# IDEA-Research/MP-Former

Measured on AMD Instinct MI355X. Metric: training images/sec COCO-instance R50 1024x1024, higher is better.
Workload: dtype bf16 (backbone, decoder) + f32 (pixel decoder, losses), as the reference's AMP; 1 GPU; COCO-instance R50, 100 queries, 80 classes, 1024x1024: full train step = R50 backbone + MSDeformAttn pixel decoder (6 layers) + MP masked decoder (9 layers, NUM_DN 1) + Hungarian matching + 60 losses + backward + grad all-reduce + clip + AdamW; head_only_workload=False, global_batch=2, per_gpu_batch=2, parallelism=dp1, msda_offsets=init, full=False, autograd_threads=backward on the launch thread, miopen_find_db=shipped

## Files before the change

### include/mpformer_hip.h

```cpp
#ifndef MPFORMER_HIP_H
#define MPFORMER_HIP_H

#include <stddef.h>
#include <stdint.h>

#ifdef __cplusplus
extern "C" {
#endif

enum { MPF_F32 = 0, MPF_F64 = 1, MPF_BF16 = 2, MPF_U8 = 3, MPF_BITS = 4  };

enum {
    MPF_OK = 0,
    MPF_E_DTYPE = -1,
    MPF_E_SHAPE = -2,
    MPF_E_NULL = -3,
    MPF_E_TOO_LARGE = -4
};

int mpf_abi_version(void);
const char* mpf_last_error(void);

int mpf_msda_forward(const void* value, const int64_t* spatial_shapes,
                     const int64_t* level_start_index, const void* sampling_loc,
// ... 244 lines not shown
    int N, Q, HW, pad;
    float eps;
} MpfNextMask;
size_t mpf_next_attn_mask_scratch_bytes(int N, int Q);
int mpf_next_attn_mask(const MpfNextMask* m, void* stream);
int mpf_decoder_layer_backward(const MpfDecoderLayer* layer, const MpfDecoderLayerGrad* grad, void* stream);

typedef struct MpfScaleCastItem {
    const void* src;
    void* dst;
    const float* scale;
    int64_t numel, inner, first_block;
} MpfScaleCastItem;

int mpf_grouped_scale_cast(const MpfScaleCastItem* items_device, int n_items, int64_t total_blocks, int src_dtype, int dst_dtype,
                           void* stream);

#define MPF_AMAX_SLOT_FLOATS 512
int mpf_res_ln256_forward_b(const float* x, const void* t, int t_dtype, const float* gamma, const float* beta, float* s_out, float* y32,
                            void* y16, float* mean, float* rstd, int rows, float eps, const float* padd, int padd_rows, float* y_plus,
                            float* y_bound, const float* padd_amax, float* yplus_bound, void* stream);
int mpf_res_ln256_backward_ws_amax(const float* s, const float* mean, const float* rstd, const float* gamma, const float* gy32,
                                   const void* gy16, const float* gy_plus, float* ds32, void* ds16, float* dgamma, float* dbeta, int rows,
                                   void* workspace, size_t workspace_bytes, float* ds_amax, void* stream);
typedef struct MpfAmaxItem {
    const float* src;
    float* out;
    int64_t numel, first_block;
} MpfAmaxItem;
typedef struct MpfSplitItemH2 {
    const float* src;
    void* dst;
    const float* amax;
    int64_t rows, cols, transpose, dst_ld, plane_stride, first_block;
} MpfSplitItemH2;
int mpf_amax_f32(const float* x, int64_t n, float* amax, void* stream);
int mpf_amax_f32_grouped(const MpfAmaxItem* items_device, int n_items, int64_t total_blocks, void* stream);
int mpf_h2_range_stats(const float* a, int rows, int cols, int64_t lda, const float* amax_slot, int log2_below,
                       unsigned long long* counters_device, void* stream);
int mpf_gemm3_split_grouped_h2(const MpfSplitItemH2* items_device, int n_items, int64_t total_blocks, void* stream);
typedef struct MpfNtItemH2 {
    const float* a;
    int64_t lda;
    const float* a_amax;
    const float* b;
    int64_t ldb;
    const float* b_amax;
    float* c_part;
    float* csum_a;
    int64_t Mdim, Ndim;
} MpfNtItemH2;
int mpf_gemm3_nt_h2(const float* a, int64_t lda, const float* a_amax, const float* b, int64_t ldb, const float* b_amax,
                    float* c_part, float* csum_a, float* csum_b, int R, int Mdim, int Ndim, int rows_per_split,
                    int transpose_out, void* stream);
int mpf_gemm3_nt_grouped_h2(const MpfNtItemH2* items, int n_items, int R, int rows_per_split, int64_t split_stride, void* stream);
int mpf_gemm3_conv3x3_h2(const float* x, const float* x_amax, const void* w_planes_h2, const float* w_amax, const float* bias,
                         float* y, float* out_amax, int n_img, int H, int W, int Cin, int Cout, int transposed, void* stream);
int mpf_gemm3_conv3x3_wgrad_h2(const float* dy, const float* dy_amax, const float* x, const float* x_amax, float* c_part,
                               float* csum_dy, int n_img, int H, int W, int Cin, int Cout, int rows_per_split, void* stream);
int mpf_gemm3_tn_h2(const float* a, int64_t lda, const float* a_amax, const void* b_planes_h2, const float* b_amax,
                    const float* bias, const float* c_in, int64_t ldcin, const float* c_in2, int64_t ldcin2,
                    const float* gate, int64_t ldgate, float* c, int64_t ldc, float* out_amax, int M, int N, int K,
                    int relu, void* stream);
int mpf_gemm3_tn_h2_bits(const float* a, int64_t lda, const float* a_amax, const void* b_planes_h2, const float* b_amax,
                         const float* bias, const float* c_in, int64_t ldcin, const float* c_in2, int64_t ldcin2,
                         const unsigned char* gate_bits, int64_t ldgbits, float* c, int64_t ldc, float* out_amax,
                         unsigned char* gate_bits_out, int64_t ldgbits_out, int M, int N, int K, int relu, void* stream);

typedef struct MpfNtItem {
    const float* a;
    int64_t lda;
    const float* b;
    int64_t ldb;
    float* c_part;
    float* csum_a;
    int64_t Mdim, Ndim;
} MpfNtItem;
int mpf_gemm3_nt_grouped(const MpfNtItem* items, int n_items, int R, int rows_per_split, int64_t split_stride, void* stream);

int mpf_gemm3_conv3x3(const float* x, const void* w_planes, const float* bias, float* y, int n_img, int H, int W, int Cin,
                      int Cout, int transposed, void* stream);
int mpf_gemm3_conv3x3_wgrad(const float* dy, const float* x, float* c_part, float* csum_dy, int n_img, int H, int W, int Cin, int Cout,
                            int rows_per_split, void* stream);

int mpf_gemm3_tn_ex(const void* a, int a_dtype, int64_t lda, const void* b_planes, const float* bias, const float* c_in, int64_t ldcin,
                    void* c, int c_dtype, int64_t ldc, int M, int N, int K, int relu, void* stream);
int mpf_gemm3_nt_ex(const void* a, int a_dtype, int64_t lda, const void* b, int b_dtype, int64_t ldb, float* c_part, float* csum_a,
                    int R, int Mdim, int Ndim, int rows_per_split, void* stream);

typedef struct MpfSplitItem {
    const float* src;
    void* dst;
    int64_t rows, cols, transpose, dst_ld, plane_stride, first_block;
} MpfSplitItem;

int mpf_gemm3_split_grouped(const MpfSplitItem* items_device, int n_items, int64_t total_blocks, void* stream);

typedef struct MpfOptItem {
    float* param;
    const float* grad;
    float* exp_avg;
    float* exp_avg_sq;
    int64_t numel, first_block;
    float lr, weight_decay, bc1, bc2_sqrt;
} MpfOptItem;

int mpf_clip_adamw_step(const MpfOptItem* items_device, int n_items, int64_t total_blocks, float max_norm, double beta1,
                        double beta2, double eps, float* partial, float* norm_clip, void* stream);

int mpf_transpose_f32(const float* in, int64_t in_batch_stride, float* out, int64_t out_batch_stride, int B, int R, int C,
                      void* stream);

int mpf_gemm3_nt_reduce(const float* c_part, int64_t c_numel, const float* s_part, int64_t s_numel, int nsplit,
                        float* c_out, float* s_out, void* stream);
int mpf_gemm3_nt_reduce_levels(const float* c_part, int64_t c_numel, const float* s_part, int64_t s_numel, int nsplit,
                               const int64_t* level_of_split, int n_levels, float* c_out, float* lvl_out, float* s_out, void* stream);

int mpf_tall_gemm_bf16(const void* a, int64_t lda, const void* b, int64_t ldb, const void* bias, void* c, int64_t ldc, int M, int N,
                       int K, void* stream);
size_t mpf_gemm_nt_bf16_workspace_bytes(int R, int Mdim, int Ndim, int rows_per_split);
int mpf_gemm_nt_bf16(const void* a, int64_t lda, const void* b, int64_t ldb, void* c_out, void* csum_out, int R, int Mdim,
                     int Ndim, int rows_per_split, void* workspace, size_t workspace_bytes, void* stream);

int mpf_small_gemm_bf16_blocked(const void* a, int64_t a_rs, int64_t a_ks, int a_blk, int64_t a_bs, const void* gate, const void* b,
                                int64_t b_rs, int64_t b_ks, const void* bias, const void* c_in, int64_t ldcin, void* c, int64_t ldc,
                                int c_blk, int64_t c_bs, void* rowsum_a, int I, int J, int Kc, int relu, void* stream);

int mpf_class_loss_forward(const void* logits, int dtype, int64_t sl, int64_t sn, int64_t sq, const int64_t* target,
                           int target_per_output, const float* weight, int L, int N, int Q, int C, float* lse, float* ce,
                           float* wsum, void* stream);
int mpf_class_loss_backward(const void* logits, int dtype, int64_t sl, int64_t sn, int64_t sq, const int64_t* target,
                            int target_per_output, const float* weight, int L, int N, int Q, int C, const float* lse,
                            const float* wsum, const float* grad_ce, void* dlogits, void* stream);
int mpf_mask_loss_finalize(const float* sums, const int64_t* runs, const float* norm, int n, int G, int points, float* out,
                           void* stream);
int mpf_mask_loss_finalize_backward(const float* sums, const int64_t* runs, const float* norm, int n, int G, int points,
                                    const float* grad_out, float* dsums, void* stream);

typedef struct {
    const void* a;
    const void* gate;
    const void* b;
    void* c;
    void* rowsum_a;
    int64_t a_rs, a_ks, a_bs, b_rs, b_ks, ldc;
    int a_blk, I, J, Kc;
} MpfSmallGemmItem;
int mpf_small_gemm_bf16_group(const MpfSmallGemmItem* items, int n_items, void* stream);
typedef struct MpfTransposeItem {
    const void* src;
    const void* gate;
    void* dst;
    int64_t ld;
    int R, C;
} MpfTransposeItem;
int mpf_transpose_group_bf16(const MpfTransposeItem* items, int n_items, int Rp, void* stream);

int mpf_bias_act(const void* x, const float* bias, const void* res, void* y, int64_t numel, int C, int dtype,
                 int relu, void* stream);
int mpf_relu_bwd_add(const void* ga, const void* gb, const void* y, void* out, int64_t numel, int dtype, void* stream);
int mpf_maxpool3x3s2_forward(const void* x, void* y, void* code, int N, int H, int W, int C, void* stream);
int mpf_maxpool3x3s2_backward(const void* gy, const void* code, void* gx, int N, int H, int W, int C, void* stream);

int mpf_upload_small(const void* host_src, void* device_dst, int64_t nbytes, void* stream);

int mpf_res_ln256_forward(const float* x, const void* t, int t_dtype, const float* gamma, const float* beta,
// ... 144 lines not shown
```

### mp_former_amd/_lib.py

```python
import ctypes

import torch
import os

_HERE = os.path.dirname(os.path.abspath(__file__))
LIB_PATH = os.path.join(_HERE, "libmpformer_hip.so")
LIB_PATH = os.environ.get("MPF_LIB_PATH", LIB_PATH)
ABI_VERSION = 1

MPF_F32, MPF_F64, MPF_BF16, MPF_U8, MPF_BITS = 0, 1, 2, 3, 4
DTYPE = {torch.float32: MPF_F32, torch.float64: MPF_F64, torch.bfloat16: MPF_BF16, torch.uint8: MPF_U8, torch.bool: MPF_U8}

_lib = None
_status_fns = {}

_c_int = ctypes.c_int
_c_vp = ctypes.c_void_p

SIGNATURES = {
    "mpf_abi_version": (_c_int, []),
    "mpf_last_error": (ctypes.c_char_p, []),
    "mpf_last_kernel": (ctypes.c_char_p, []),
    "mpf_set_option": (_c_int, [ctypes.c_char_p, _c_int]),
    "mpf_match_cost_fused_workspace_bytes": (ctypes.c_size_t, [_c_int] * 5),
# ... 49 lines not shown
    "mpf_amax_f32": (_c_int, [_c_vp, ctypes.c_int64, _c_vp, _c_vp]),
    "mpf_amax_f32_grouped": (_c_int, [_c_vp, _c_int, ctypes.c_int64, _c_vp]),
    "mpf_h2_range_stats": (_c_int, [_c_vp, _c_int, _c_int, ctypes.c_int64, _c_vp, _c_int, _c_vp, _c_vp]),
    "mpf_gemm3_split_grouped_h2": (_c_int, [_c_vp, _c_int, ctypes.c_int64, _c_vp]),
    "mpf_gemm3_tn_h2": (_c_int, [_c_vp, ctypes.c_int64, _c_vp, _c_vp, _c_vp, _c_vp, _c_vp, ctypes.c_int64, _c_vp, ctypes.c_int64,
                              _c_vp, ctypes.c_int64, _c_vp, ctypes.c_int64, _c_vp, _c_int, _c_int, _c_int, _c_int, _c_vp]),
    "mpf_gemm3_tn_h2_bits": (_c_int, [_c_vp, ctypes.c_int64, _c_vp, _c_vp, _c_vp, _c_vp, _c_vp, ctypes.c_int64, _c_vp, ctypes.c_int64,
                                   _c_vp, ctypes.c_int64, _c_vp, ctypes.c_int64, _c_vp, _c_vp, ctypes.c_int64,
                                   _c_int, _c_int, _c_int, _c_int, _c_vp]),
    "mpf_gemm3_nt_h2": (_c_int, [_c_vp, ctypes.c_int64, _c_vp, _c_vp, ctypes.c_int64, _c_vp, _c_vp, _c_vp, _c_vp,
                              _c_int, _c_int, _c_int, _c_int, _c_int, _c_vp]),
    "mpf_gemm3_nt_grouped_h2": (_c_int, [_c_vp, _c_int, _c_int, _c_int, ctypes.c_int64, _c_vp]),
    "mpf_gemm3_conv3x3_h2": (_c_int, [_c_vp] * 7 + [_c_int] * 6 + [_c_vp]),
    "mpf_gemm3_conv3x3_wgrad_h2": (_c_int, [_c_vp, _c_vp, _c_vp, _c_vp, _c_vp, _c_vp, _c_int, _c_int, _c_int, _c_int, _c_int, _c_int, _c_vp]),
    "mpf_gemm3_nt_grouped": (_c_int, [_c_vp, _c_int, _c_int, _c_int, ctypes.c_int64, _c_vp]),
    "mpf_small_gemm_bf16": (_c_int, [_c_vp, ctypes.c_int64, ctypes.c_int64, _c_vp, _c_vp, ctypes.c_int64, ctypes.c_int64, _c_vp, _c_vp,
                                     ctypes.c_int64, _c_vp, ctypes.c_int64, _c_vp, _c_int, _c_int, _c_int, _c_int, _c_vp]),
    "mpf_encoder_fields": (_c_int, []),
    "mpf_encoder_forward": (_c_int, [_c_vp, _c_vp]),
    "mpf_encoder_bwd_fields": (_c_int, []),
    "mpf_encoder_backward": (_c_int, [_c_vp, _c_vp]),
    "mpf_decoder_layer_struct_bytes": (ctypes.c_uint64, [_c_int]),
    "mpf_decoder_layer_scratch_bytes": (ctypes.c_uint64, [_c_int] * 6),
    "mpf_decoder_layer_forward": (_c_int, [_c_vp, _c_vp]),
    "mpf_next_attn_mask_scratch_bytes": (ctypes.c_size_t, [_c_int, _c_int]),
    "mpf_next_attn_mask": (_c_int, [_c_vp, _c_vp]),
    "mpf_lin256_res_ln_forward": (_c_int, [_c_vp] * 11 + [_c_int, ctypes.c_float, _c_vp]),
    "mpf_ln256_mlp3_forward": (_c_int, [_c_vp] * 10 + [_c_int, ctypes.c_float, _c_vp]),
    "mpf_decoder_layer_backward": (_c_int, [_c_vp, _c_vp, _c_vp]),
    "mpf_pool_features": (_c_int, [_c_vp, _c_int, _c_vp] + [_c_int] * 6 + [_c_vp]),
    "mpf_pool_features_cl": (_c_int, [_c_vp, ctypes.c_int64, _c_int, _c_vp, _c_int, _c_int, _c_int, _c_int, _c_int, _c_int, _c_vp]),
    "mpf_mask_head_bits": (_c_int, [_c_vp, ctypes.c_int64, ctypes.c_int64, _c_vp, _c_vp, _c_int, _c_vp, _c_vp] + [_c_int] * 3 + [_c_vp]),
    "mpf_lsa_assign": (_c_int, [_c_vp, _c_vp, _c_int, _c_int, ctypes.c_int64] + [_c_vp] * 7),
    "mpf_lsa_assign_status": (_c_int, [_c_vp, _c_vp, _c_int, _c_int, ctypes.c_int64] + [_c_vp] * 8),
    "mpf_mask_block_empty": (_c_int, [_c_vp, _c_vp] + [_c_int] * 5 + [_c_vp]),
    "mpf_mp_open_counts": (_c_int, [_c_vp, _c_int, _c_int, _c_vp, _c_vp]),
    "mpf_mp_noise_rows": (_c_int, [_c_vp] * 3 + [_c_int] * 4 + [ctypes.c_double, ctypes.c_uint64, ctypes.c_uint64, _c_vp, _c_vp]),
    "mpf_gemm_nt_bf16_workspace_bytes": (ctypes.c_size_t, [_c_int] * 4),
    "mpf_gemm_nt_bf16": (_c_int, [_c_vp, ctypes.c_int64, _c_vp, ctypes.c_int64, _c_vp, _c_vp, _c_int, _c_int, _c_int, _c_int, _c_vp,
                                  ctypes.c_size_t, _c_vp]),
    "mpf_gemm3_nt_reduce": (_c_int, [_c_vp, ctypes.c_int64, _c_vp, ctypes.c_int64, _c_int, _c_vp, _c_vp, _c_vp]),
    "mpf_grouped_scale_cast": (_c_int, [_c_vp, _c_int, ctypes.c_int64, _c_int, _c_int, _c_vp]),
    "mpf_gemm3_split_grouped": (_c_int, [_c_vp, _c_int, ctypes.c_int64, _c_vp]),
    "mpf_decoder_inputs_forward": (_c_int, [_c_vp, ctypes.c_int64, ctypes.c_int64, _c_vp, _c_vp, _c_vp, _c_vp, _c_int, _c_int, _c_int, _c_int,
                                            _c_vp]),
    "mpf_decoder_inputs_backward": (_c_int, [_c_vp, _c_vp, _c_int, _c_vp, ctypes.c_int64, ctypes.c_int64, _c_int, _c_int, _c_int, _c_vp]),
    "mpf_clip_adamw_step": (_c_int, [_c_vp, _c_int, ctypes.c_int64, ctypes.c_float, ctypes.c_double, ctypes.c_double, ctypes.c_double,
                                     _c_vp, _c_vp, _c_vp]),
    "mpf_transpose_f32": (_c_int, [_c_vp, ctypes.c_int64, _c_vp, ctypes.c_int64, _c_int, _c_int, _c_int, _c_vp]),
    "mpf_small_gemm_bf16_blocked": (_c_int, [_c_vp, ctypes.c_int64, ctypes.c_int64, _c_int, ctypes.c_int64, _c_vp, _c_vp, ctypes.c_int64,
                                             ctypes.c_int64, _c_vp, _c_vp, ctypes.c_int64, _c_vp, ctypes.c_int64, _c_int, ctypes.c_int64,
                                             _c_vp, _c_int, _c_int, _c_int, _c_int, _c_vp]),
    "mpf_small_gemm_bf16_group": (_c_int, [_c_vp, _c_int, _c_vp]),
    "mpf_transpose_group_bf16": (_c_int, [_c_vp, _c_int, _c_int, _c_vp]),
    "mpf_class_loss_forward": (_c_int, [_c_vp, _c_int, ctypes.c_int64, ctypes.c_int64, ctypes.c_int64, _c_vp, _c_int, _c_vp, _c_int, _c_int,
                                        _c_int, _c_int, _c_vp, _c_vp, _c_vp, _c_vp]),
    "mpf_class_loss_backward": (_c_int, [_c_vp, _c_int, ctypes.c_int64, ctypes.c_int64, ctypes.c_int64, _c_vp, _c_int, _c_vp, _c_int, _c_int,
                                         _c_int, _c_int, _c_vp, _c_vp, _c_vp, _c_vp, _c_vp]),
    "mpf_mask_loss_finalize": (_c_int, [_c_vp, _c_vp, _c_vp, _c_int, _c_int, _c_int, _c_vp, _c_vp]),
    "mpf_mask_loss_finalize_backward": (_c_int, [_c_vp, _c_vp, _c_vp, _c_int, _c_int, _c_int, _c_vp, _c_vp, _c_vp]),
    "mpf_bias_act": (_c_int, [_c_vp, _c_vp, _c_vp, _c_vp, ctypes.c_int64, _c_int, _c_int, _c_int, _c_vp]),
    "mpf_relu_bwd_add": (_c_int, [_c_vp, _c_vp, _c_vp, _c_vp, ctypes.c_int64, _c_int, _c_vp]),
    "mpf_maxpool3x3s2_forward": (_c_int, [_c_vp] * 3 + [_c_int] * 4 + [_c_vp]),
    "mpf_maxpool3x3s2_backward": (_c_int, [_c_vp] * 3 + [_c_int] * 4 + [_c_vp]),
    "mpf_upload_small": (_c_int, [_c_vp, _c_vp, ctypes.c_int64, _c_vp]),
    "mpf_tall_gemm_bf16": (_c_int, [_c_vp, ctypes.c_int64, _c_vp, ctypes.c_int64, _c_vp, _c_vp, ctypes.c_int64, _c_int, _c_int, _c_int, _c_vp]),
    "mpf_res_ln256_forward": (_c_int, [_c_vp, _c_vp, _c_int, _c_vp, _c_vp, _c_vp, _c_vp, _c_vp, _c_vp, _c_vp, _c_int, ctypes.c_float,
                                       _c_vp, _c_int, _c_vp, _c_vp]),
    "mpf_res_ln256_forward_b": (_c_int, [_c_vp, _c_vp, _c_int, _c_vp, _c_vp, _c_vp, _c_vp, _c_vp, _c_vp, _c_vp, _c_int, ctypes.c_float,
                                         _c_vp, _c_int, _c_vp, _c_vp, _c_vp, _c_vp, _c_vp]),
    "mpf_res_ln256_backward_ws_amax": (_c_int, [_c_vp] * 11 + [_c_int, _c_vp, ctypes.c_size_t, _c_vp, _c_vp]),
    "mpf_res_ln256_backward": (_c_int, [_c_vp] * 11 + [_c_int, _c_vp]),
    "mpf_mask_loss_backward_dense": (_c_int, [_c_vp, _c_int, _c_int, _c_int, _c_vp, _c_vp, _c_int, _c_int, _c_int, _c_vp, _c_vp, _c_vp,
                                              _c_vp, _c_int, _c_vp, _c_int, _c_int, _c_vp]),
    "mpf_gn_cl_supported": (_c_int, [_c_int, _c_int, _c_int]),
    "mpf_gn_cl_workspace_bytes": (ctypes.c_size_t, [_c_int, _c_int, _c_int, _c_int]),
    "mpf_gn_cl_forward": (_c_int, [_c_vp, ctypes.c_int64, _c_vp, _c_vp, _c_int, _c_int, _c_int, _c_int, ctypes.c_float, _c_int,
                                   _c_vp, ctypes.c_int64, _c_int, _c_vp, ctypes.c_int64, _c_vp, _c_vp, _c_vp, ctypes.c_size_t, _c_vp]),
    "mpf_gn_cl_backward": (_c_int, [_c_vp, ctypes.c_int64, _c_vp, ctypes.c_int64, _c_vp, _c_vp, _c_vp, _c_vp, _c_int, _c_int, _c_int,
                                    _c_int, _c_int, _c_vp, ctypes.c_int64, _c_vp, _c_vp, _c_vp, ctypes.c_size_t, _c_vp]),
    "mpf_upsample2x_cl_backward": (_c_int, [_c_vp, ctypes.c_int64, _c_int, _c_int, _c_int, _c_int, _c_vp, ctypes.c_int64, _c_vp]),
    "mpf_gemm3_conv3x3": (_c_int, [_c_vp, _c_vp, _c_vp, _c_vp, _c_int, _c_int, _c_int, _c_int, _c_int, _c_int, _c_vp]),
    "mpf_gemm3_conv3x3_wgrad": (_c_int, [_c_vp, _c_vp, _c_vp, _c_vp, _c_int, _c_int, _c_int, _c_int, _c_int, _c_int, _c_vp]),
    "mpf_gemm3_nt_reduce_levels": (_c_int, [_c_vp, ctypes.c_int64, _c_vp, ctypes.c_int64, _c_int, _c_vp, _c_int, _c_vp, _c_vp, _c_vp, _c_vp]),
    "mpf_gemm3_tn_ex": (_c_int, [_c_vp, _c_int, ctypes.c_int64, _c_vp, _c_vp, _c_vp, ctypes.c_int64, _c_vp, _c_int, ctypes.c_int64,
                                 _c_int, _c_int, _c_int, _c_int, _c_vp]),
    "mpf_gemm3_nt_ex": (_c_int, [_c_vp, _c_int, ctypes.c_int64, _c_vp, _c_int, ctypes.c_int64, _c_vp, _c_vp, _c_int, _c_int, _c_int, _c_int, _c_vp]),
    "mpf_res_ln256_backward_workspace_bytes": (ctypes.c_size_t, [_c_int]),
    "mpf_res_ln256_backward_partial": (_c_int, [_c_vp] * 9 + [_c_int, _c_vp, ctypes.c_size_t, _c_vp]),
    "mpf_res_ln256_backward_partial_amax": (_c_int, [_c_vp] * 9 + [_c_int, _c_vp, ctypes.c_size_t, _c_vp, _c_vp]),
    "mpf_ln_partial_reduce": (_c_int, [_c_vp, ctypes.c_size_t, _c_int, _c_int, _c_vp, _c_vp]),
    "mpf_res_ln256_backward_det_workspace_bytes": (ctypes.c_size_t, [_c_int]),
    "mpf_res_ln256_backward_det": (_c_int, [_c_vp] * 10 + [_c_int, _c_vp, ctypes.c_size_t, _c_vp]),
    "mpf_res_ln256_backward_ws": (_c_int, [_c_vp] * 11 + [_c_int, _c_vp, ctypes.c_size_t, _c_vp]),
    "mpf_group_stats_workspace_bytes": (ctypes.c_size_t, [_c_int, ctypes.c_int64]),
    "mpf_group_stats": (_c_int, [_c_vp, _c_int, ctypes.c_int64, ctypes.c_float, _c_vp, _c_vp, _c_vp, ctypes.c_size_t, _c_vp]),
    "mpf_msda_forward": (_c_int, [_c_vp] * 6 + [_c_int] * 8 + [_c_vp]),
    "mpf_msda_backward": (_c_int, [_c_vp] * 9 + [_c_int] * 8 + [_c_vp]),
    "mpf_msda_forward_hs": (_c_int, [_c_vp] * 7 + [_c_int] * 8 + [_c_vp]),
    "mpf_msda_forward_raw_hs": (_c_int, [_c_vp] * 9 + [_c_int] * 8 + [_c_vp]),
    "mpf_msda_forward_raw": (_c_int, [_c_vp] * 8 + [_c_int] * 8 + [_c_vp]),
    "mpf_msda_backward_ws_raw": (_c_int, [_c_vp] * 7 + [_c_int] * 8 + [_c_vp, ctypes.c_size_t, _c_vp]),
    "mpf_msda_backward_ws_raw_o": (_c_int, [_c_vp] * 8 + [_c_int] * 8 + [_c_vp, ctypes.c_size_t, _c_vp, _c_vp, _c_vp]),
    "mpf_msda_backward_workspace_bytes": (ctypes.c_size_t, [_c_int] * 5 + [_c_vp]),
    "mpf_msda_backward_ws": (_c_int, [_c_vp] * 8 + [_c_int] * 8 + [_c_vp, ctypes.c_size_t, _c_vp]),
    "mpf_seg_softmax": (_c_int, [_c_vp, _c_int, _c_int, ctypes.c_float] + [_c_vp] * 6),
    "mpf_seg_semantic": (_c_int, [_c_vp, ctypes.c_int64] + [_c_int] * 10 + [_c_vp, _c_int, _c_vp, _c_vp]),
    "mpf_seg_instance_workspace_bytes": (ctypes.c_size_t, [_c_int] * 3),
    "mpf_seg_instance_scores": (_c_int, [_c_vp, ctypes.c_int64] + [_c_int] * 10 + [_c_vp, _c_vp, _c_int, _c_vp, _c_vp, ctypes.c_size_t,
                                                                                   _c_vp]),
    "mpf_seg_instance_masks": (_c_int, [_c_vp, ctypes.c_int64] + [_c_int] * 10 + [_c_vp, _c_int, _c_vp, _c_vp]),
    "mpf_seg_panoptic_areas": (_c_int, [_c_vp, ctypes.c_int64] + [_c_int] * 10 + [_c_vp] * 5),
    "mpf_seg_panoptic_paint": (_c_int, [_c_vp, _c_int, _c_int, _c_vp, _c_vp, _c_vp]),
    "mpf_seg_semantic_labels": (_c_int, [_c_vp, ctypes.c_int64] + [_c_int] * 10 + [_c_vp, _c_int, _c_vp, _c_vp]),
    "mpf_seg_labels_resize": (_c_int, [_c_vp] + [_c_int] * 5 + [_c_vp, _c_vp]),
    "mpf_seg_confusion_add": (_c_int, [_c_vp, _c_vp, ctypes.c_int64, _c_int, _c_int, _c_vp, _c_vp]),
    "mpf_seg_instance_rle_workspace_bytes": (ctypes.c_size_t, [_c_int] * 3),
    "mpf_seg_instance_rle_count": (_c_int, [_c_vp, ctypes.c_int64] + [_c_int] * 10 + [_c_vp, _c_int, _c_vp, _c_vp, ctypes.c_size_t, _c_vp]),
    "mpf_seg_instance_rle_write": (_c_int, [_c_vp, ctypes.c_size_t, _c_int, _c_int, _c_int, _c_vp, ctypes.c_int64, _c_vp, _c_vp, _c_vp]),
}


class NativeLibraryError(RuntimeError):
    pass


def lib():
    global _lib
    if _lib is None:
        if not os.path.exists(LIB_PATH):
            raise NativeLibraryError(
                f"{LIB_PATH} not found: build it with `python -c 'import __graft_entry__ as g; g.build()'` "
                "or `make -C mp_former_amd/csrc`.  mp_former_amd has no CPU / eager fallback.")
        l = ctypes.CDLL(LIB_PATH)
        for name, (res, args) in SIGNATURES.items():
            try:
                fn = getattr(l, name)
            except AttributeError as e:
                raise NativeLibraryError(f"{LIB_PATH} does not export {name}") from e
            fn.restype = res
            fn.argtypes = args
            if res is _c_int:
                _status_fns[name] = fn
        v = l.mpf_abi_version()
        if v != ABI_VERSION:
            raise NativeLibraryError(f"ABI mismatch: library {v}, binding {ABI_VERSION}")
        _lib = l
        for kv in filter(None, os.environ.get("MPF_OPTIONS", "").split(",")):
            k, _, v = kv.partition("=")
            set_option(k.strip(), int(v))
    return _lib


def check(code, what):
    if code != 0:
        msg = lib().mpf_last_error().decode()
        raise RuntimeError(f"{what} failed with code {code}: {msg}")


def _status_fn(name):
    lib()
    fn = _status_fns.get(name)
    if fn is None:
        raise TypeError(f"{name} does not return a status: call() is for the int-returning entry points, sizes go through lib()")
    return fn

# ... 92 lines not shown
```

### mp_former_amd/backbone.py

```python
import numpy as np
import torch
import torch.nn.functional as F
from torch import nn

from . import _lib
from ._h2d import upload


class FrozenBatchNorm2d(nn.Module):

    def __init__(self, num_features, eps=1e-5):
        super().__init__()
        self.eps = eps
        self.register_buffer("weight", torch.ones(num_features))
        self.register_buffer("bias", torch.zeros(num_features))
        self.register_buffer("running_mean", torch.zeros(num_features))
        self.register_buffer("running_var", torch.ones(num_features))

    def scale_bias(self):
        b = self._buffers
        w, bb, rm, rv = b["weight"], b["bias"], b["running_mean"], b["running_var"]
        c = self.__dict__.get("_sb_cache")
        if (c is None or c[0] is not w or c[1] is not bb or c[2] is not rm or c[3] is not rv
                or c[4] != (w._version, bb._version, rm._version, rv._version)):
            with torch.no_grad():
                scale = w * (rv + self.eps).rsqrt()
                c = (w, bb, rm, rv, (w._version, bb._version, rm._version, rv._version), scale,
                     (bb - rm * scale).float().contiguous())
            self.__dict__["_sb_cache"] = c
        return c[5], c[6]

    def forward(self, x):
        scale, bias = self.scale_bias()
        return x * scale.to(x.dtype).view(1, -1, 1, 1) + bias.to(x.dtype).view(1, -1, 1, 1)


class _BiasAct(torch.autograd.Function):

    @staticmethod
    def forward(ctx, x, shift, res, relu):
        y = torch.empty_like(x)
        C = x.shape[1]
        _lib.call("mpf_bias_act", x.device, x.data_ptr(), shift.data_ptr(), _lib.ptr(res), y.data_ptr(), x.numel(), C,
                  _lib.DTYPE[x.dtype], 1 if relu else 0, _lib.stream_ptr(x.device))
        ctx.relu, ctx.has_res = relu, res is not None
        if relu:
            ctx.save_for_backward(y)
        return y

    @staticmethod
    def backward(ctx, g):
        if ctx.relu:
            (y,) = ctx.saved_tensors
            g = torch.ops.aten.threshold_backward(g, y, 0)
        return g, None, (g if ctx.has_res else None), None


def _relu_bwd_add(ga, gb, y):
    same = (ga.dtype == torch.bfloat16 and y.dtype == torch.bfloat16 and ga.shape == y.shape and ga.stride() == y.stride() and _dense(y)
            and ga.numel() % 8 == 0 and (gb is None or (gb.dtype == ga.dtype and gb.shape == ga.shape and gb.stride() == ga.stride())))
    if not (ga.is_cuda and same):
        return torch.ops.aten.threshold_backward(ga if gb is None else ga + gb, y, 0)
    out = torch.empty_like(y)
    _lib.call("mpf_relu_bwd_add", y.device, ga.data_ptr(), _lib.ptr(gb), y.data_ptr(), out.data_ptr(), y.numel(), _lib.MPF_BF16,
              _lib.stream_ptr(y.device))
    return out


class _BiasActFork(torch.autograd.Function):

    @staticmethod
    def forward(ctx, x, shift, res):
        y = torch.empty_like(x)
        _lib.call("mpf_bias_act", x.device, x.data_ptr(), shift.data_ptr(), res.data_ptr(), y.data_ptr(), x.numel(), x.shape[1],
                  _lib.DTYPE[x.dtype], 1, _lib.stream_ptr(x.device))
        ctx.save_for_backward(y)
        ctx.set_materialize_grads(False)
        return y, y.view(y.shape)

    @staticmethod
    def backward(ctx, ga, gb):
        (y,) = ctx.saved_tensors
        if ga is None and gb is None:
            return None, None, None
        if ga is None:
            ga, gb = gb, None
        g = _relu_bwd_add(ga, gb, y)
        return g, None, g


def _bias_act_ok(x, res):
    return (x.is_cuda and x.dim() == 4 and x.dtype in (torch.bfloat16, torch.float32) and x.shape[1] % 8 == 0
            and x.is_contiguous(memory_format=torch.channels_last)
            and (res is None or (res.dtype == x.dtype and res.shape == x.shape
                                 and res.is_contiguous(memory_format=torch.channels_last))))


def bias_act(x, shift, res=None, relu=True):
    if _bias_act_ok(x, res):
        return _BiasAct.apply(x, shift, res, relu)
    y = x + shift.to(x.dtype).view(1, -1, 1, 1)
    if res is not None:
        y = y + res
    return F.relu(y) if relu else y


def bias_act_fork(x, shift, res):
    if _bias_act_ok(x, res) and x.dtype == torch.bfloat16:
        return _BiasActFork.apply(x, shift, res)
    y = bias_act(x, shift, res, True)
    return y, y


class _MaxPool3x3s2(torch.autograd.Function):

    @staticmethod
    def forward(ctx, x):
        N, C, H, W = x.shape
        OH, OW = (H - 1) // 2 + 1, (W - 1) // 2 + 1
        y = torch.empty((N, C, OH, OW), dtype=x.dtype, device=x.device, memory_format=torch.channels_last)
        code = torch.empty((N, OH, OW, C), dtype=torch.uint8, device=x.device)
        _lib.call("mpf_maxpool3x3s2_forward", x.device, x.data_ptr(), y.data_ptr(), code.data_ptr(), N, H, W, C,
                  _lib.stream_ptr(x.device))
        ctx.save_for_backward(code)
        ctx.in_shape = (N, C, H, W)
        return y

    @staticmethod
    def backward(ctx, gy):
        (code,) = ctx.saved_tensors
        N, C, H, W = ctx.in_shape
        if gy.dtype != torch.bfloat16 or not gy.is_contiguous(memory_format=torch.channels_last):
            gy = gy.to(torch.bfloat16).contiguous(memory_format=torch.channels_last)
        gx = torch.empty((N, C, H, W), dtype=gy.dtype, device=gy.device, memory_format=torch.channels_last)
        _lib.call("mpf_maxpool3x3s2_backward", gy.device, gy.data_ptr(), code.data_ptr(), gx.data_ptr(), N, H, W, C,
                  _lib.stream_ptr(gy.device))
        return gx


def max_pool_3x3_s2(x):
    if (x.is_cuda and x.dim() == 4 and x.dtype == torch.bfloat16 and x.shape[1] % 8 == 0 and 256 % (x.shape[1] // 8) == 0
            and x.is_contiguous(memory_format=torch.channels_last)):
        return _MaxPool3x3s2.apply(x)
    return F.max_pool2d(x, kernel_size=3, stride=2, padding=1)


def conv_bn(conv, bn, x, folded=None, res=None, relu=True, fork=False):
    if folded is not None:
        w, shift = folded
    else:
        scale, shift = bn.scale_bias()
        w = conv.weight * scale.view(-1, 1, 1, 1)
    y = F.conv2d(x, w, None, conv.stride, conv.padding, conv.dilation, conv.groups)
    return bias_act_fork(y, shift, res) if fork else bias_act(y, shift, res, relu)


def _dense(t):
    return t.is_contiguous() or (t.dim() == 4 and t.is_contiguous(memory_format=torch.channels_last))


_gsc_layouts = {}


def _grouped_scale_cast(srcs, scales, out_dtype):
    dev = srcs[0].device
    key = tuple([(t.shape, t.stride()) for t in srcs] + [id(sc) for sc in scales] + [out_dtype])
    lay = _gsc_layouts.get(key)
    if lay is None:
        numels = [t.numel() for t in srcs]
        offs, tot, blk = [], 0, 0
        table = np.zeros((len(srcs), 6), dtype=np.int64)
        for i, (t, sc) in enumerate(zip(srcs, scales)):
            assert _dense(t) and sc.dtype == torch.float32 and sc.is_contiguous() and sc.numel() == t.shape[0]
            offs.append(tot)
            table[i, 2:] = (sc.data_ptr(), numels[i], numels[i] // t.shape[0], blk)
            tot += (numels[i] + 63) & ~63
            blk += (numels[i] + 2047) // 2048
        esz = torch.empty(0, dtype=out_dtype).element_size()
        lay = (table, np.asarray(offs, dtype=np.int64) * esz, tot, blk, [(o, n, t.shape, t.stride()) for o, n, t in zip(offs, numels, srcs)],
               list(scales))
        if len(_gsc_layouts) > 64:
            _gsc_layouts.clear()
        _gsc_layouts[key] = lay
    table, offs_b, tot, blk, views, _ = lay
    out = torch.empty(tot, dtype=out_dtype, device=dev)
    table[:, 0] = [t.data_ptr() for t in srcs]
    table[:, 1] = offs_b + out.data_ptr()
    items = upload(table.reshape(-1), dev)
    _lib.call("mpf_grouped_scale_cast", dev, items.data_ptr(), len(srcs), blk, _lib.DTYPE[srcs[0].dtype], _lib.DTYPE[out_dtype],
              _lib.stream_ptr(dev))
    return [out[o:o + n].as_strided(shp, std) for o, n, shp, std in views]


class _FoldCast(torch.autograd.Function):

    @staticmethod
    def forward(ctx, dtype, scales, *weights):
        ctx.scales = scales
        ws = [p.detach() for p in weights]
        native = (ws[0].is_cuda and all(w.dtype == torch.float32 and _dense(w) for w in ws)
                  and dtype in (None, torch.float32, torch.bfloat16))
        ctx.native = native
        if native:
            return tuple(_grouped_scale_cast(ws, scales, dtype or torch.float32))
        w = torch._foreach_mul(ws, [s_.view(-1, 1, 1, 1) for s_ in scales])
        if dtype is None:
            return tuple(w)
        outs = [torch.empty_like(t, dtype=dtype) for t in w]
        torch._foreach_copy_(outs, w)
        return tuple(outs)

    @staticmethod
    def backward(ctx, *grads):
        if ctx.native and all(g is not None and g.dtype == grads[0].dtype for g in grads) \
                and grads[0].dtype in (torch.float32, torch.bfloat16):
            gs = [g if _dense(g) else g.contiguous() for g in grads]
            return (None, None, *_grouped_scale_cast(gs, ctx.scales, torch.float32))
        g32 = [torch.empty_like(g, dtype=torch.float32) for g in grads]
        torch._foreach_copy_(g32, list(grads))
        torch._foreach_mul_(g32, [s_.view(-1, 1, 1, 1) for s_ in ctx.scales])
        return (None, None, *g32)


_PAIR_NAMES = (("conv1", "norm1"), ("conv2", "norm2"), ("conv3", "norm3"), ("shortcut", "shortcut_norm"))


class Bottleneck(nn.Module):
    def __init__(self, cin, cmid, cout, stride):
        super().__init__()
        self.shortcut = None
        if cin != cout or stride != 1:
            self.shortcut = nn.Conv2d(cin, cout, 1, stride=stride, bias=False)
            self.shortcut_norm = FrozenBatchNorm2d(cout)
        self.conv1 = nn.Conv2d(cin, cmid, 1, bias=False)
        self.norm1 = FrozenBatchNorm2d(cmid)
        self.conv2 = nn.Conv2d(cmid, cmid, 3, stride=stride, padding=1, bias=False)
# ... 84 lines not shown
```

### mp_former_amd/csrc/common.hip

```cpp
#include "mpf_common.h"

#include <stdio.h>

#include <atomic>
#include <mutex>
#include <string>
#include <vector>

namespace {
thread_local char t_err[256] = "";
std::atomic<const char*> g_kernel{""};
}

namespace mpf {
int fail(int code, const char* msg)
{
    snprintf(t_err, sizeof(t_err), "%s", msg);
    return code;
}

int check(hipError_t err, const char* where)
{
    if (err == hipSuccess) return 0;
    snprintf(t_err, sizeof(t_err), "%s: %s (%d)", where, hipGetErrorString(err), (int)err);
// ... 35 lines not shown

extern "C" int mpf_profile_enable(int on)
{
    std::lock_guard<std::mutex> lk(mpf::g_prof_mu);
    for (auto& r : mpf::g_prof) { (void)hipEventDestroy(r.e0); (void)hipEventDestroy(r.e1); }
    mpf::g_prof.clear();
    mpf::g_prof_on.store(on ? 1 : 0);
    return 0;
}

extern "C" int mpf_profile_get(const char* name_substr, int* count, double* total_ms, double* total_bytes)
{
    if (!name_substr || !count || !total_ms || !total_bytes) return MPF_E_NULL;
    std::lock_guard<std::mutex> lk(mpf::g_prof_mu);
    int n = 0; double ms = 0, by = 0;
    for (auto& r : mpf::g_prof) {
        if (!strstr(r.name, name_substr)) continue;
        if (hipEventSynchronize(r.e1) != hipSuccess) continue;
        float t = 0.f;
        if (hipEventElapsedTime(&t, r.e0, r.e1) != hipSuccess) continue;
        ms += t; by += r.bytes; ++n;
    }
    *count = n; *total_ms = ms; *total_bytes = by;
    return 0;
}

extern "C" int mpf_profile_get_flops(const char* name_substr, double* total_flops)
{
    if (!name_substr || !total_flops) return MPF_E_NULL;
    std::lock_guard<std::mutex> lk(mpf::g_prof_mu);
    double fl = 0;
    for (auto& r : mpf::g_prof)
        if (strstr(r.name, name_substr)) fl += r.flops;
    *total_flops = fl;
    return 0;
}

namespace {
constexpr int kUpPayload = 3968;
struct UpPayload { uint32_t w[kUpPayload / 4]; };
__global__ __launch_bounds__(256) void upload_small_kernel(UpPayload p, uint32_t* __restrict__ dst, int nwords)
{
    for (int i = threadIdx.x; i < nwords; i += 256) dst[i] = p.w[i];
}
}

extern "C" int mpf_upload_small(const void* host_src, void* device_dst, int64_t nbytes, void* stream)
{
    if (nbytes == 0) return 0;
    if (!host_src || !device_dst) return mpf::fail(MPF_E_NULL, "upload_small: NULL buffer");
    if (nbytes < 0 || (nbytes & 3) || ((uintptr_t)device_dst & 3)) return mpf::fail(MPF_E_SHAPE, "upload_small: size / destination must be multiples of 4 bytes");
    const unsigned char* src = static_cast<const unsigned char*>(host_src);
    unsigned char* dst = static_cast<unsigned char*>(device_dst);
    for (int64_t off = 0; off < nbytes; off += kUpPayload) {
        const int n = (int)((nbytes - off) < kUpPayload ? (nbytes - off) : kUpPayload);
        UpPayload p;
        memcpy(p.w, src + off, (size_t)n);
        hipLaunchKernelGGL(upload_small_kernel, dim3(1), dim3(256), 0, (hipStream_t)stream, p, reinterpret_cast<uint32_t*>(dst + off), n / 4);
    }
    return mpf::check(hipGetLastError(), "mpf_upload_small");
}

extern "C" int mpf_abi_version(void) { return 1; }
extern "C" const char* mpf_last_error(void) { return t_err; }
extern "C" const char* mpf_last_kernel(void) { return g_kernel.load(std::memory_order_relaxed); }

extern "C" int mpf_set_option(const char* key, int value)
{
    if (!key) return MPF_E_NULL;
    int r = mpf::set_msda_option(key, value);
    if (r <= 0) return r;
    r = mpf::set_binned_option(key, value);
    if (r <= 0) return r;
    r = mpf::set_gemm3_option(key, value);
    if (r <= 0) return r;
    r = mpf::set_decoder_option(key, value);
    if (r <= 0) return r;
    r = mpf::set_block_option(key, value);
    if (r <= 0) return r;
    r = mpf::set_attn_option(key, value);
    if (r <= 0) return r;
    r = mpf::set_small_gemm_option(key, value);
    if (r <= 0) return r;
    return mpf::fail(MPF_E_SHAPE, "mpf_set_option: unknown key");
}
```

### mp_former_amd/csrc/mpf_common.h

```cpp
#pragma once
#include <hip/hip_runtime.h>
#include <string.h>

#include <atomic>

#include "../../include/mpformer_hip.h"

namespace mpf {
int fail(int code, const char* msg);
int check(hipError_t err, const char* where);
void set_kernel(const char* name);
void prof_begin(hipStream_t st);
void prof_end(const char* name, hipStream_t st, double algorithmic_bytes, double flops = 0.0);
constexpr int kMaxDevices = 32;
struct LdsAttr { std::atomic<int> bytes[kMaxDevices] = {}; };
inline int ensure_dynamic_lds(const void* fn, size_t bytes, LdsAttr& slots)
{
    int dev = 0;
    if (hipGetDevice(&dev) != hipSuccess || dev < 0 || dev >= kMaxDevices) dev = -1;
    if (dev >= 0 && slots.bytes[dev].load(std::memory_order_relaxed) >= (int)bytes) return 0;
    if (int e = check(hipFuncSetAttribute(fn, hipFuncAttributeMaxDynamicSharedMemorySize, (int)bytes), "hipFuncSetAttribute")) return e;
    if (dev >= 0) slots.bytes[dev].store((int)bytes, std::memory_order_relaxed);
    return 0;
}
inline int cu_count()
{
    static std::atomic<int> cache[kMaxDevices];
    int dev = 0, cus = 0;
    if (hipGetDevice(&dev) != hipSuccess || dev < 0 || dev >= kMaxDevices) return 256;
    cus = cache[dev].load(std::memory_order_relaxed);
    if (cus > 0) return cus;
    if (hipDeviceGetAttribute(&cus, hipDeviceAttributeMultiprocessorCount, dev) != hipSuccess || cus <= 0) cus = 256;
    cache[dev].store(cus, std::memory_order_relaxed);
    return cus;
}
int set_msda_option(const char* key, int v);
int set_binned_option(const char* key, int v);
int set_gemm3_option(const char* key, int v);
int set_block_option(const char* key, int v);
int set_decoder_option(const char* key, int v);
int set_attn_option(const char* key, int v);
int set_small_gemm_option(const char* key, int v);
int msda_block_forward(const void* value, const int64_t* host_shapes, const void* loc, const void* attn, void* out, int N, int S, int M,
                       int D, int L, int Lq, int P, int dtype, hipStream_t st, const void* raw = nullptr, const void* ref = nullptr);
size_t msda_block_workspace_bytes(const int64_t* host_shapes, int N, int M, int L, int Lq, int P);
int msda_block_backward(const void* value, const int64_t* host_shapes, const void* loc, const void* attn, const void* go, void* gv,
                        void* gl, void* ga, void* graw, int N, int S, int M, int D, int L, int Lq, int P, int dtype, void* workspace,
                        size_t workspace_bytes, hipStream_t st, const void* fwd_out = nullptr, float* graw_amax = nullptr,
                        float* gv_amax = nullptr, bool* amax_recorded = nullptr);
}
```

Measured before the change: 86.93 images/sec.

## Add native bf16 MFMA weight-gradient kernel for ResNet 3x3 backbone convs

```diff
diff --git a/include/mpformer_hip.h b/include/mpformer_hip.h
--- a/include/mpformer_hip.h
+++ b/include/mpformer_hip.h
@@ -350,6 +350,10 @@
                       int Cout, int transposed, void* stream);
 int mpf_gemm3_conv3x3_wgrad(const float* dy, const float* x, float* c_part, float* csum_dy, int n_img, int H, int W, int Cin, int Cout,
                             int rows_per_split, void* stream);
+int mpf_conv_wgrad_bf16_supported(int Cin, int Cout, int H, int W, int stride);
+size_t mpf_conv_wgrad_bf16_workspace_bytes(int n_img, int H, int W, int C, int stride);
+int mpf_conv_wgrad_bf16(const void* dy, const void* x, void* dw, int n_img, int H, int W, int C, int stride, void* workspace,
+                        size_t workspace_bytes, void* stream);
 
 int mpf_gemm3_tn_ex(const void* a, int a_dtype, int64_t lda, const void* b_planes, const float* bias, const float* c_in, int64_t ldcin,
                     void* c, int c_dtype, int64_t ldc, int M, int N, int K, int relu, void* stream);
diff --git a/mp_former_amd/_lib.py b/mp_former_amd/_lib.py
--- a/mp_former_amd/_lib.py
+++ b/mp_former_amd/_lib.py
@@ -155,6 +155,9 @@
     "mpf_upsample2x_cl_backward": (_c_int, [_c_vp, ctypes.c_int64, _c_int, _c_int, _c_int, _c_int, _c_vp, ctypes.c_int64, _c_vp]),
     "mpf_gemm3_conv3x3": (_c_int, [_c_vp, _c_vp, _c_vp, _c_vp, _c_int, _c_int, _c_int, _c_int, _c_int, _c_int, _c_vp]),
     "mpf_gemm3_conv3x3_wgrad": (_c_int, [_c_vp, _c_vp, _c_vp, _c_vp, _c_int, _c_int, _c_int, _c_int, _c_int, _c_int, _c_vp]),
+    "mpf_conv_wgrad_bf16_supported": (_c_int, [_c_int] * 5),
+    "mpf_conv_wgrad_bf16_workspace_bytes": (ctypes.c_size_t, [_c_int] * 5),
+    "mpf_conv_wgrad_bf16": (_c_int, [_c_vp] * 3 + [_c_int] * 5 + [_c_vp, ctypes.c_size_t, _c_vp]),
     "mpf_gemm3_nt_reduce_levels": (_c_int, [_c_vp, ctypes.c_int64, _c_vp, ctypes.c_int64, _c_int, _c_vp, _c_int, _c_vp, _c_vp, _c_vp, _c_vp]),
     "mpf_gemm3_tn_ex": (_c_int, [_c_vp, _c_int, ctypes.c_int64, _c_vp, _c_vp, _c_vp, ctypes.c_int64, _c_vp, _c_int, ctypes.c_int64,
                                  _c_int, _c_int, _c_int, _c_int, _c_vp]),
diff --git a/mp_former_amd/backbone.py b/mp_former_amd/backbone.py
--- a/mp_former_amd/backbone.py
+++ b/mp_former_amd/backbone.py
@@ -1,3 +1,5 @@
+import os
+
 import numpy as np
 import torch
 import torch.nn.functional as F
@@ -145,13 +147,80 @@
     return F.max_pool2d(x, kernel_size=3, stride=2, padding=1)
 
 
+_WGRAD_NATIVE = int(os.environ.get("MPF_CONV_WGRAD_NATIVE", "1"))
+_WGRAD_ROUTES = frozenset({(64, 1), (128, 1), (128, 2), (256, 1), (256, 2), (512, 1), (512, 2)})
+_wgrad_plans = {}
+
+
+def _wgrad_plan(N, C, H, W, stride):
+    key = (N, C, H, W, stride, _lib.option_generation())
+    nbytes = _wgrad_plans.get(key)
+    if nbytes is None:
+        l = _lib.lib()
+        nbytes = l.mpf_conv_wgrad_bf16_workspace_bytes(N, H, W, C, stride) if l.mpf_conv_wgrad_bf16_supported(C, C, H, W, stride) else 0
+        if len(_wgrad_plans) > 64:
+            _wgrad_plans.clear()
+        _wgrad_plans[key] = nbytes
+    return nbytes
+
+
+def conv3x3_wgrad_native(gy, x, w_like, stride, nbytes):
+    N, C, H, W = x.shape
+    dw = torch.empty_like(w_like)
+    st = _lib.stream_ptr(x.device)
+    ws = _lib.scratch("conv_wgrad_bf16", x.device, st, nbytes)
+    _lib.call("mpf_conv_wgrad_bf16", x.device, gy.data_ptr(), x.data_ptr(), dw.data_ptr(), N, H, W, C, stride, ws.data_ptr(),
+              ws.numel(), st)
+    return dw
+
+
+class _Conv3x3NativeWgrad(torch.autograd.Function):
+
+    @staticmethod
+    def forward(ctx, x, w, stride, nbytes):
+        ctx.save_for_backward(x, w)
+        ctx.stride, ctx.nbytes = stride, nbytes
+        return torch.ops.aten.convolution(x, w, None, [stride, stride], [1, 1], [1, 1], False, [0, 0], 1)
+
+    @staticmethod
+    def backward(ctx, gy):
+        x, w = ctx.saved_tensors
+        s = ctx.stride
+        gx = gw = None
+        if not gy.is_contiguous(memory_format=torch.channels_last):
+            gy = gy.contiguous(memory_format=torch.channels_last)
+        if ctx.needs_input_grad[0]:
+            gx = torch.ops.aten.convolution_backward(gy, x, w, None, [s, s], [1, 1], [1, 1], False, [0, 0], 1, [True, False, False])[0]
+        if ctx.needs_input_grad[1]:
+            gw = conv3x3_wgrad_native(gy, x, w, s, ctx.nbytes)
+        return gx, gw, None, None
+
+
+def _wgrad_native_bytes(conv, x, w):
+    if conv.kernel_size != (3, 3) or not (_WGRAD_NATIVE and w.requires_grad and x.is_cuda and torch.is_grad_enabled()):
+        return 0
+    if not (x.dtype == torch.bfloat16 and w.dtype == torch.bfloat16 and x.dim() == 4
+            and conv.padding == (1, 1) and conv.dilation == (1, 1) and conv.groups == 1 and conv.stride in ((1, 1), (2, 2))
+            and w.shape[0] == w.shape[1] == x.shape[1]
+            and x.is_contiguous(memory_format=torch.channels_last) and w.is_contiguous(memory_format=torch.channels_last)):
+        return 0
+    N, C, H, W = x.shape
+    if _WGRAD_NATIVE < 2 and (C, conv.stride[0]) not in _WGRAD_ROUTES:
+        return 0
+    return _wgrad_plan(N, C, H, W, conv.stride[0])
+
+
 def conv_bn(conv, bn, x, folded=None, res=None, relu=True, fork=False):
     if folded is not None:
         w, shift = folded
     else:
         scale, shift = bn.scale_bias()
         w = conv.weight * scale.view(-1, 1, 1, 1)
-    y = F.conv2d(x, w, None, conv.stride, conv.padding, conv.dilation, conv.groups)
+    nbytes = _wgrad_native_bytes(conv, x, w)
+    if nbytes:
+        y = _Conv3x3NativeWgrad.apply(x, w, conv.stride[0], nbytes)
+    else:
+        y = F.conv2d(x, w, None, conv.stride, conv.padding, conv.dilation, conv.groups)
     return bias_act_fork(y, shift, res) if fork else bias_act(y, shift, res, relu)
 
 
diff --git a/mp_former_amd/csrc/common.hip b/mp_former_amd/csrc/common.hip
--- a/mp_former_amd/csrc/common.hip
+++ b/mp_former_amd/csrc/common.hip
@@ -141,5 +141,7 @@
     if (r <= 0) return r;
     r = mpf::set_small_gemm_option(key, value);
     if (r <= 0) return r;
+    r = mpf::set_conv_wgrad_option(key, value);
+    if (r <= 0) return r;
     return mpf::fail(MPF_E_SHAPE, "mpf_set_option: unknown key");
 }
diff --git a/mp_former_amd/csrc/conv_wgrad_bf16.hip b/mp_former_amd/csrc/conv_wgrad_bf16.hip
--- /dev/null
+++ b/mp_former_amd/csrc/conv_wgrad_bf16.hip
@@ -0,0 +1,245 @@
+#include "mpf_common.h"
+
+namespace {
+
+typedef short s4v __attribute__((ext_vector_type(4)));
+typedef short s8v __attribute__((ext_vector_type(8)));
+typedef __bf16 bf8v __attribute__((ext_vector_type(8)));
+typedef float f16v __attribute__((ext_vector_type(16)));
+typedef unsigned u4v __attribute__((ext_vector_type(4)));
+
+constexpr int kTile = 64;
+constexpr int kStepPx = 32;
+constexpr int kPY = 192;
+
+__device__ __attribute__((aligned(256))) unsigned g_zero_row[32];
+
+int g_target_wgs = 512;
+
+struct Params {
+    const unsigned short* dy;
+    const unsigned short* x;
+    float* part;
+    int H, W, OH, OW, C;
+    int nsplit, steps_per_split, steps;
+};
+
+__device__ __forceinline__ bf8v tr_pair(const unsigned char* lo, const unsigned char* hi)
+{
+    typedef s4v __attribute__((address_space(3))) * lds_p;
+    const s4v a = __builtin_amdgcn_ds_read_tr16_b64_v4i16((lds_p)lo);
+    const s4v b = __builtin_amdgcn_ds_read_tr16_b64_v4i16((lds_p)hi);
+    return __builtin_bit_cast(bf8v, __builtin_shufflevector(a, b, 0, 1, 2, 3, 4, 5, 6, 7));
+}
+
+template <int S>
+__global__ __launch_bounds__(256) void conv_wgrad_bf16_kernel(const Params p)
+{
+    constexpr int PX = S == 1 ? 192 : 160;
+    constexpr int NPX = kStepPx * S + 2;
+    constexpr int RX = (NPX * 8 + 255) / 256;
+    constexpr int XB = RX * 32 * PX, YB = kStepPx * kPY;
+    __shared__ __attribute__((aligned(16))) unsigned char lds_x[2 * XB];
+    __shared__ __attribute__((aligned(16))) unsigned char lds_y[2 * YB];
+
+    const int tid = threadIdx.x, l = tid & 63, w = tid >> 6, wm = w & 1, wn = w >> 1;
+    const int split = blockIdx.x % p.nsplit;
+    int tile = blockIdx.x / p.nsplit;
+    const int ky = tile % 3;
+    tile /= 3;
+    const int tc = p.C / kTile;
+    const int ci0 = (tile % tc) * kTile, co0 = (tile / tc) * kTile;
+    const int C = p.C, H = p.H, W = p.W, OH = p.OH, OW = p.OW, nxb = OW / kStepPx;
+
+    const int t0 = split * p.steps_per_split;
+    const int t1 = min(t0 + p.steps_per_split, p.steps);
+    int oxb = t0 % nxb, oy = (t0 / nxb) % OH, n = (t0 / nxb) / OH, tl = t0;
+
+    const int lpx = tid >> 3, lch = tid & 7;
+    const int64_t zoff = reinterpret_cast<const unsigned char*>(g_zero_row) - reinterpret_cast<const unsigned char*>(p.x) + lch * 16;
+
+    auto load = [&](u4v& ry, u4v(&rx)[RX]) __attribute__((always_inline)) {
+        const int ox0 = oxb * kStepPx;
+        ry = *reinterpret_cast<const u4v*>(p.dy + ((size_t)(n * OH + oy) * OW + ox0 + lpx) * C + co0 + lch * 8);
+        const int iy = oy * S + ky - 1;
+        const bool rowok = (unsigned)iy < (unsigned)H;
+        const int64_t xrow = ((int64_t)(n * H + (rowok ? iy : 0)) * W * C + ci0 + lch * 8) * 2;
+#pragma unroll
+        for (int r = 0; r < RX; ++r) {
+            const int px = lpx + 32 * r;
+            const int ix = S * ox0 - 1 + px;
+            const bool ok = rowok && (unsigned)ix < (unsigned)W && px < NPX;
+            const int64_t off = ok ? xrow + (int64_t)(ix * C * 2) : zoff;
+            rx[r] = *reinterpret_cast<const u4v*>(reinterpret_cast<const unsigned char*>(p.x) + off);
+        }
+        if (tl + 1 < t1) {
+            ++tl;
+            if (++oxb == nxb) {
+                oxb = 0;
+                if (++oy == OH) { oy = 0; ++n; }
+            }
+        }
+    };
+    auto store = [&](int buf, const u4v& ry, const u4v(&rx)[RX]) __attribute__((always_inline)) {
+        *reinterpret_cast<u4v*>(lds_y + buf * YB + lpx * kPY + lch * 16) = ry;
+#pragma unroll
+        for (int r = 0; r < RX; ++r) *reinterpret_cast<u4v*>(lds_x + buf * XB + (lpx + 32 * r) * PX + lch * 16) = rx[r];
+    };
+
+    const int kh = l >> 5, g1 = (l >> 4) & 1, q = (l >> 2) & 3, j4 = l & 3;
+    const int a_off = (8 * kh + q) * kPY + (32 * wm + 16 * g1 + 4 * j4) * 2;
+    const int b_off = S * (8 * kh + q) * PX + (32 * wn + 16 * g1 + 4 * j4) * 2;
+
+    f16v acc[3];
+#pragma unroll
+    for (int k = 0; k < 3; ++k)
+#pragma unroll
+        for (int r = 0; r < 16; ++r) acc[k][r] = 0.f;
+
+    u4v ry1, rx1[RX], ry2, rx2[RX];
+    load(ry1, rx1);
+    store(0, ry1, rx1);
+    load(ry1, rx1);
+    __syncthreads();
+
+    auto step = [&](int buf, u4v& ry_nxt, u4v(&rx_nxt)[RX], u4v& ry_far, u4v(&rx_far)[RX]) __attribute__((always_inline)) {
+        load(ry_far, rx_far);
+        const unsigned char* ya = lds_y + buf * YB + a_off;
+        const unsigned char* xb = lds_x + buf * XB + b_off;
+#pragma unroll
+        for (int kk = 0; kk < 2; ++kk) {
+            const bf8v a = tr_pair(ya + (16 * kk) * kPY, ya + (16 * kk + 4) * kPY);
+#pragma unroll
+            for (int kx = 0; kx < 3; ++kx) {
+                const bf8v b = tr_pair(xb + (S * 16 * kk + kx) * PX, xb + (S * (16 * kk + 4) + kx) * PX);
+                acc[kx] = __builtin_amdgcn_mfma_f32_32x32x16_bf16(a, b, acc[kx], 0, 0, 0);
+            }
+        }
+        store(buf ^ 1, ry_nxt, rx_nxt);
+        __syncthreads();
+    };
+    for (int t = t0; t + 1 < t1; t += 2) {
+        step(0, ry1, rx1, ry2, rx2);
+        step(1, ry2, rx2, ry1, rx1);
+    }
+    if ((t1 - t0) & 1) step(0, ry1, rx1, ry2, rx2);
+
+    float* pp = p.part + (size_t)split * 9 * C * C;
+    const int ci = ci0 + 32 * wn + (l & 31);
+#pragma unroll
+    for (int kx = 0; kx < 3; ++kx)
+#pragma unroll
+        for (int r = 0; r < 16; ++r) {
+            const int co = co0 + 32 * wm + (r & 3) + 8 * (r >> 2) + 4 * kh;
+            pp[((size_t)(co * 3 + ky) * 3 + kx) * C + ci] = acc[kx][r];
+        }
+}
+
+__global__ __launch_bounds__(256) void conv_wgrad_bf16_reduce_kernel(const float* __restrict__ part, int numel, int nsplit,
+                                                                     unsigned* __restrict__ out)
+{
+    const int j = blockIdx.x * 256 + threadIdx.x;
+    if (j >= numel / 2) return;
+    const float* src = part + 2 * (size_t)j;
+    float2 acc = make_float2(0.f, 0.f);
+    int sp = 0;
+    for (; sp + 8 <= nsplit; sp += 8) {
+        float2 t[8];
+#pragma unroll
+        for (int k = 0; k < 8; ++k) t[k] = *reinterpret_cast<const float2*>(src + (size_t)(sp + k) * numel);
+#pragma unroll
+        for (int k = 0; k < 8; ++k) { acc.x += t[k].x; acc.y += t[k].y; }
+    }
+    for (; sp < nsplit; ++sp) {
+        const float2 t = *reinterpret_cast<const float2*>(src + (size_t)sp * numel);
+        acc.x += t.x; acc.y += t.y;
+    }
+    auto rne = [](float f) -> unsigned {
+        unsigned u = __float_as_uint(f);
+        if ((u & 0x7fffffffu) > 0x7f800000u) return (u >> 16) | 0x40u;
+        u += 0x7fffu + ((u >> 16) & 1u);
+        return u >> 16;
+    };
+    out[j] = rne(acc.x) | (rne(acc.y) << 16);
+}
+
+struct Plan { int OH, OW, steps, nsplit, steps_per_split; };
+
+bool make_plan(int n_img, int H, int W, int C, int stride, Plan& pl)
+{
+    if (!(C == 64 || C == 128 || C == 256 || C == 512) || (stride != 1 && stride != 2) || n_img < 1 || H < 1 || W < 1) return false;
+    pl.OH = (H - 1) / stride + 1;
+    pl.OW = (W - 1) / stride + 1;
+    if (pl.OW % kStepPx) return false;
+    if ((int64_t)n_img * H * W * C >= (int64_t)1 << 31) return false;
+    pl.steps = n_img * pl.OH * (pl.OW / kStepPx);
+    const int tiles = (C / kTile) * (C / kTile) * 3;
+    int ns = (g_target_wgs + tiles - 1) / tiles;
+    if (ns >= 8) ns = (ns + 7) & ~7;
+    if (ns > pl.steps) ns = pl.steps;
+    pl.steps_per_split = (pl.steps + ns - 1) / ns;
+    pl.nsplit = (pl.steps + pl.steps_per_split - 1) / pl.steps_per_split;
+    return true;
+}
+
+}
+
+namespace mpf {
+int set_conv_wgrad_option(const char* key, int v)
+{
+    if (!strcmp(key, "conv_wgrad_wgs")) {
+        if (v < 1 || v > 65536) return fail(MPF_E_SHAPE, "mpf_set_option: conv_wgrad_wgs must be in 1..65536");
+        g_target_wgs = v;
+        return 0;
+    }
+    return 1;
+}
+}
+
+extern "C" int mpf_conv_wgrad_bf16_supported(int Cin, int Cout, int H, int W, int stride)
+{
+    Plan pl;
+    return Cin == Cout && make_plan(1, H, W, Cin, stride, pl) ? 1 : 0;
+}
+
+extern "C" size_t mpf_conv_wgrad_bf16_workspace_bytes(int n_img, int H, int W, int C, int stride)
+{
+    Plan pl;
+    if (!make_plan(n_img, H, W, C, stride, pl)) return 0;
+    return (size_t)pl.nsplit * 9 * C * C * sizeof(float);
+}
+
+extern "C" int mpf_conv_wgrad_bf16(const void* dy, const void* x, void* dw, int n_img, int H, int W, int C, int stride,
+                                   void* workspace, size_t workspace_bytes, void* stream)
+{
+    if (!dy || !x || !dw || !workspace) return mpf::fail(MPF_E_NULL, "conv_wgrad_bf16: NULL buffer");
+    Plan pl;
+    if (!make_plan(n_img, H, W, C, stride, pl))
+        return mpf::fail(MPF_E_SHAPE, "conv_wgrad_bf16: needs Cin == Cout in {64, 128, 256, 512}, stride 1 or 2, output width % 32 == 0 "
+                                      "(mpf_conv_wgrad_bf16_supported)");
+    if (workspace_bytes < (size_t)pl.nsplit * 9 * C * C * sizeof(float))
+        return mpf::fail(MPF_E_SHAPE, "conv_wgrad_bf16: workspace smaller than mpf_conv_wgrad_bf16_workspace_bytes");
+    if (((uintptr_t)dy | (uintptr_t)x | (uintptr_t)workspace) & 15 || ((uintptr_t)dw & 3))
+        return mpf::fail(MPF_E_SHAPE, "conv_wgrad_bf16: dy, x, workspace must be 16-byte aligned, dw 4-byte aligned");
+    hipStream_t st = (hipStream_t)stream;
+    Params p;
+    p.dy = static_cast<const unsigned short*>(dy);
+    p.x = static_cast<const unsigned short*>(x);
+    p.part = static_cast<float*>(workspace);
+    p.H = H; p.W = W; p.OH = pl.OH; p.OW = pl.OW; p.C = C;
+    p.nsplit = pl.nsplit; p.steps_per_split = pl.steps_per_split; p.steps = pl.steps;
+    const int tiles = (C / kTile) * (C / kTile) * 3, numel = 9 * C * C;
+    const double flops = 2.0 * numel * (double)n_img * pl.OH * pl.OW;
+    const double bytes = 2.0 * n_img * ((double)H * W + (double)pl.OH * pl.OW) * C + 4.0 * numel * pl.nsplit;
+    mpf::prof_begin(st);
+    mpf::set_kernel("conv_wgrad_bf16_kernel");
+    if (stride == 1)
+        hipLaunchKernelGGL(conv_wgrad_bf16_kernel<1>, dim3((unsigned)(tiles * pl.nsplit)), dim3(256), 0, st, p);
+    else
+        hipLaunchKernelGGL(conv_wgrad_bf16_kernel<2>, dim3((unsigned)(tiles * pl.nsplit)), dim3(256), 0, st, p);
+    mpf::prof_end("conv_wgrad_bf16_kernel", st, bytes, flops);
+    if (int e = mpf::check(hipGetLastError(), "mpf_conv_wgrad_bf16")) return e;
+    hipLaunchKernelGGL(conv_wgrad_bf16_reduce_kernel, dim3((unsigned)((numel / 2 + 255) / 256)), dim3(256), 0, st, p.part, numel,
+                       pl.nsplit, static_cast<unsigned*>(dw));
+    return mpf::check(hipGetLastError(), "mpf_conv_wgrad_bf16 (reduce)");
+}
diff --git a/mp_former_amd/csrc/mpf_common.h b/mp_former_amd/csrc/mpf_common.h
--- a/mp_former_amd/csrc/mpf_common.h
+++ b/mp_former_amd/csrc/mpf_common.h
@@ -41,6 +41,7 @@
 int set_decoder_option(const char* key, int v);
 int set_attn_option(const char* key, int v);
 int set_small_gemm_option(const char* key, int v);
+int set_conv_wgrad_option(const char* key, int v);
 int msda_block_forward(const void* value, const int64_t* host_shapes, const void* loc, const void* attn, void* out, int N, int S, int M,
                        int D, int L, int Lq, int P, int dtype, hipStream_t st, const void* raw = nullptr, const void* ref = nullptr);
 size_t msda_block_workspace_bytes(const int64_t* host_shapes, int N, int M, int L, int Lq, int P);
```

After: 87.88 images/sec, median of 4. No clear change (+1.1%).
